# jayleicn/TVRetrieval

Hardware: AMD Instinct MI355X
Metric: queries/sec VCMR over 21.8K-video corpus (higher is better)
Workload: dtype bf16

## Files before the change

### include/xmlhip.h

```cpp
#ifndef XMLHIP_H
#define XMLHIP_H

#include <stddef.h>
#include <stdint.h>

#ifdef __cplusplus
extern "C" {
#endif

typedef void* xml_stream_t;

typedef enum { XML_F32 = 0, XML_BF16 = 1, XML_F16 = 2, XML_F16S = 3 } xml_dtype;
#define XML_F16_UNIT_LOG2 14

typedef enum {
  XML_OK = 0,
  XML_ERR_BAD_ARG = -1,
  XML_ERR_UNSUPPORTED = -2,
  XML_ERR_WORKSPACE = -3,
  XML_ERR_LAUNCH = -4
} xml_status;

int xml_abi_version(void);
const char* xml_build_arch(void);
// ... 239 lines not shown
                                    xml_stream_t stream);
int xml_q2c_scores_arg(const void* qn, const void* cn, const float* mask, float* out, int64_t ld_out, int32_t* arg,
                       int64_t ld_arg, int nq, int nv, int l, int hidden, int combine, int dt, xml_stream_t stream);
int xml_loss_combine(const float* st_ed, const float* rank2, float w_st_ed, float w_neg_ctx, float w_neg_q, float* parts4,
                     float* overall, xml_stream_t stream);
int xml_loss_combine_bwd(const float* g, float w_st_ed, float w_neg_ctx, float w_neg_q, float* d_st_ed, float* d_rank2,
                         xml_stream_t stream);
int xml_pair_sim(const void* q, const void* f2, float* sim, int64_t n, int l, int hidden, int dt,
                 xml_stream_t stream);
int xml_pair_sim_bwd(const void* q, const void* f2, const float* dsim, void* dq, void* df2, int64_t n, int l,
                     int hidden, int dt, xml_stream_t stream);
int xml_span_loss(const float* sim0, const float* sim1, const float* conv_w, const float* mask0,
                  const float* mask1, const int64_t* st_ed, int merged, int n_sim, int ks, int n, int l,
                  const float* gout, float* loss_out, float* dsim0, float* dsim1, float* dconv_w,
                  xml_stream_t stream);
int xml_rank_loss(const float* scores, const int* ranks_ctx, const int* ranks_q, float margin, int lse,
                  int n, const float* gout, float* losses, float* dscores, xml_stream_t stream);
int xml_dropout(const void* x, void* y, int64_t n, float p, uint64_t seed, const uint64_t* seed_dev, int dt,
                xml_stream_t stream);
int xml_transpose_segments(const float* src, const int64_t* table, int n_ent, int max_tiles, int dt, xml_stream_t stream);
int xml_add_layernorm_drop(const void* a, int a_dt, const void* b, const float* g, const float* beta, void* y,
                           int64_t rows, int d, int dt, float p_in, uint64_t seed_in, float p_out, uint64_t seed_out,
                           const uint64_t* seed_dev, xml_stream_t stream);
int xml_layernorm_bwd_drop(const void* a, int a_dt, const void* b, const float* g, const void* dy, void* dx, void* dxa,
                           float* dg, float* dbeta, int64_t rows, int d, int dt, float p_in, uint64_t seed_in, float p_out,
                           uint64_t seed_out, const uint64_t* seed_dev, xml_stream_t stream);
size_t xml_layernorm_bwd_partials_bytes(int64_t rows, int d);
int xml_layernorm_bwd_drop_ws(const void* a, int a_dt, const void* b, const float* g, const void* dy, void* dx, void* dxa,
                              float* dg, float* dbeta, int64_t rows, int d, int dt, float p_in, uint64_t seed_in, float p_out,
                              uint64_t seed_out, const uint64_t* seed_dev, void* ws, size_t ws_bytes, xml_stream_t stream);
int xml_clip_grad_norm(float* g, int64_t n, float max_norm, float* ws, xml_stream_t stream);
#define XML_ADAM_NORM_BLOCK 1024
int xml_bert_adam_step(float* p, float* g, float* m, float* v, const int64_t* seg_off, const float* seg_lr,
                       const float* seg_wd, int n_seg, int64_t total, float lr_mult, float b1, float b2,
                       float eps, float max_grad_norm, float* norms, const uint8_t* seg_active,
                       const float* seg_lr_mult, float* norm_ws, xml_stream_t stream);

typedef void* xml_comm_t;
int xml_rccl_available(void);
int xml_rccl_unique_id(void* id128);
int xml_rccl_comm_init(xml_comm_t* comm, int nranks, int rank, const void* id128);
int xml_rccl_comm_destroy(xml_comm_t comm);
int xml_rccl_allgather(xml_comm_t comm, const void* send, void* recv, int64_t bytes_per_rank, xml_stream_t stream);
int xml_rccl_allreduce_avg_f32(xml_comm_t comm, float* buf, int64_t n, xml_stream_t stream);
size_t xml_rccl_allgather_topk_workspace_bytes(int world, int nq, int c);
int xml_rccl_allgather_topk(xml_comm_t comm, int world, const float* loc_score, const int32_t* loc_id, int nq, int c,
                            int k, float alpha, float* out_val, int32_t* out_id, void* ws, size_t ws_bytes,
                            xml_stream_t stream);
size_t xml_rccl_topk_by_owner_workspace_bytes(int world, int per, int c);
int xml_rccl_topk_by_owner(xml_comm_t comm, int world, int rank, const float* loc_score, const int32_t* loc_id,
                           int nq, int c, int k, float alpha, float* own_val, int32_t* own_id, void* ws,
                           size_t ws_bytes, xml_stream_t stream);

size_t xml_merge_shard_topk_workspace_bytes(int world, int n_rows, int c);
int xml_merge_shard_topk(const float* recv_score, const int32_t* recv_id, int world, int n_rows, int c, int k, float alpha,
                         float* out_val, int32_t* out_id, void* ws, size_t ws_bytes, xml_stream_t stream);

int xml_index_put_rows(int n_mod, const void* f1_a, const void* f2_a, const float* mask_a, const void* f1_b,
                       const void* f2_b, const float* mask_b, const int32_t* slots, const int32_t* ids, int b, int lb,
                       void* k6_a, void* feat2_a, float* imask_a, int32_t* bits_a, void* k6_b, void* feat2_b,
                       float* imask_b, int32_t* bits_b, int32_t* vlen, int32_t* slot_ids, int32_t* live, int capacity,
                       int lpad, int l_ref, int hidden, int dt, int tiled, xml_stream_t stream);
int xml_index_clear_rows(int n_mod, const int32_t* slots, int n, float* imask_a, int32_t* bits_a, float* imask_b,
                         int32_t* bits_b, int32_t* vlen, int32_t* live, int capacity, int lpad, int l_ref,
                         xml_stream_t stream);

int xml_nms_vcmr_host(const int64_t* vid, const double* st, const double* ed, const double* score, int n,
                      double thd, int max_before, int max_after, int32_t* out_index, int32_t* n_out);
int xml_nms_svmr_host(const double* st, const double* ed, const double* score, int n, double thd,
                      int max_before, int max_after, int32_t* out_index, int32_t* n_out);
int xml_nms_vcmr_batched_host(const int64_t* vid, const double* st, const double* ed, const double* score,
                              const int32_t* count, int nq, int64_t ld, double thd, int max_before, int max_after,
                              int32_t* out_index, int64_t ld_out, int32_t* out_count, int n_threads);
int xml_nms_svmr_batched_host(const double* st, const double* ed, const double* score, const int32_t* count, int nq,
                              int64_t ld, double thd, int max_before, int max_after, int32_t* out_index, int64_t ld_out,
                              int32_t* out_count, int n_threads);

typedef enum { XML_GEMM_SMALL = 0, XML_GEMM_256 = 1, XML_GEMM_256P = 2 } xml_gemm_kernel;
typedef enum {
  XML_GEMM_FEW = 1,
  XML_GEMM_256_OK = 2,
  XML_GEMM_256P_OK = 4,
  XML_GEMM_LN_FUSED = 8,
  XML_GEMM_TILE32 = 32, XML_GEMM_TILE64 = 64, XML_GEMM_TILE128 = 128
} xml_gemm_rules;
typedef enum { XML_KLOOP_PLAIN = 1, XML_KLOOP_DEEP2 = 2, XML_KLOOP_DEEP3 = 3 } xml_gemm_kloop;
typedef enum { XML_Q2C_UNSUPPORTED = 0, XML_Q2C_STAGED = 1, XML_Q2C_RING = 2, XML_Q2C_PERSIST = 3, XML_Q2C_NONE = 4 } xml_q2c_kernel;
typedef enum { XML_Q2C_WALK_QSH = 0, XML_Q2C_WALK_TILES_PER_WORKGROUP = 1, XML_Q2C_WALK_RING_SLOTS = 2 } xml_q2c_walk;
typedef enum {
  XML_ATTN_SMALL = 0, XML_ATTN_LARGE = 1, XML_ATTN_REFUSED_HEADS = 2, XML_ATTN_REFUSED_LENGTH = 3,
  XML_ATTN_REFUSED_LDS = 4, XML_ATTN_REFUSED_DH = 5
} xml_attn_kernel;
typedef enum { XML_L2N_SCALAR = 0, XML_L2N_VEC16 = 1 } xml_l2norm_kernel;
typedef enum {
  XML_DC_SLICE_BYTES = 0,
  XML_DC_RING_SLOTS,
  XML_DC_RING_SLOTS_NOMASK,
  XML_DC_RING_LEAD,
  XML_DC_LDS_BYTES,
  XML_DC_GEMM_FEW_TILES, XML_DC_GEMM256P_MIN_TILES, XML_DC_GEMM_LN_MIN_ROWS, XML_DC_GEMM_MIN_K_BYTES,
  XML_DC_GEMM256_MIN_M, XML_DC_GEMM256_MIN_N,
  XML_DC_GEMM_TILE128_MIN_WG, XML_DC_GEMM_TILE64_MIN_WG,
  XML_DC_Q2C_PERSIST_MIN_K_BYTES,
  XML_DC_L2N_MAXJ, XML_DC_L2N_LANES,
  XML_DC_ATTN_MAX_L, XML_DC_ATTN_SMALL_MAX_L, XML_DC_ATTN_SMALL_UNITS,
  XML_DC_ATTN_N_HEAD_SIZES, XML_DC_ATTN_HEAD_SIZE0
} xml_dispatch_constant;
int64_t xml_dispatch_const(int which);
int xml_dispatch_gemm(int64_t M, int N, int K, int dt);
int xml_dispatch_gemm_rules(int64_t M, int N, int K, int dt);
int xml_dispatch_gemm_kloop(int K, int dt, int tile);
int xml_dispatch_q2c(int lpad, int hidden, int dt, int combine);
int xml_dispatch_q2c_fused(int n_mod, int lpad, int hidden, int dt, int launch);
int xml_dispatch_q2c_walk(int what, int a, int b);
int xml_dispatch_attention(int lq, int lk, int hidden, int n_heads, int dt);
int xml_dispatch_l2norm(int d, int dt);

#ifdef __cplusplus
}
#endif
#endif
```

### tvretrieval_amd/csrc/api.hip

```cpp
#include "common.h"

extern "C" int xml_abi_version(void) {
  return 6; }
extern "C" const char* xml_build_arch(void) { return "gfx950"; }
extern "C" const char* xml_status_string(int status) {
  switch (status) {
    case XML_OK: return "ok";
    case XML_ERR_BAD_ARG: return "bad argument";
    case XML_ERR_UNSUPPORTED: return "unsupported shape";
    case XML_ERR_WORKSPACE: return "workspace too small";
    case XML_ERR_LAUNCH: return "kernel launch failed";
    default: return "unknown status";
  }
}

extern "C" int64_t xml_dispatch_const(int which) {
  namespace d = dispatch;
  static const int64_t v[] = {
      d::SLICE_BYTES, d::RING_SLOTS, d::RING_SLOTS_NOMASK, d::RING_LEAD, d::LDS_BYTES, d::GEMM_FEW_TILES, d::GEMM256P_MIN_TILES,
      d::GEMM_LN_MIN_ROWS, d::GEMM_MIN_K_BYTES, d::GEMM256_MIN_M, d::GEMM256_MIN_N, d::GEMM_TILE128_MIN_WG, d::GEMM_TILE64_MIN_WG,
      d::Q2C_PERSIST_MIN_K_BYTES, d::L2N_MAXJ, d::L2N_LANES, d::ATTN_MAX_L, d::ATTN_SMALL_MAX_L, d::ATTN_SMALL_UNITS,
      d::ATTN_N_HEAD_SIZES};
  static_assert(sizeof(v) / sizeof(v[0]) == XML_DC_ATTN_HEAD_SIZE0, "one value per xml_dispatch_constant");
  if (which >= 0 && which < XML_DC_ATTN_HEAD_SIZE0) return v[which];
  const int i = which - XML_DC_ATTN_HEAD_SIZE0;
  return i >= 0 && i < d::ATTN_N_HEAD_SIZES ? d::ATTN_HEAD_SIZES[i] : -1;
}
static bool gemm_args_ok(int64_t M, int N, int K, int dt) {
  return M > 0 && N > 0 && K > 0 && (dt == XML_F32 || dt == XML_BF16 || dt == XML_F16S);
}
extern "C" int xml_dispatch_gemm(int64_t M, int N, int K, int dt) {
  return gemm_args_ok(M, N, K, dt) ? (int)dispatch::gemm_kernel(M, N, K, dt) : -1;
}
extern "C" int xml_dispatch_gemm_rules(int64_t M, int N, int K, int dt) {
  if (!gemm_args_ok(M, N, K, dt)) return -1;
  const int tile = dispatch::gemm_small_tile(M, N);
  if (dt == XML_F16S) return tile | (dispatch::gemm256_f16s_ok(M, N, 3 * K) ? XML_GEMM_256_OK : 0);
  return tile | (dispatch::gemm_few(M, N) ? XML_GEMM_FEW : 0) | (dispatch::gemm256_ok(M, N, K, dt) ? XML_GEMM_256_OK : 0) |
         (dispatch::gemm256p_ok(M, N, K, dt) ? XML_GEMM_256P_OK : 0) | (dispatch::gemm_ln_fused(M, N, K, dt) ? XML_GEMM_LN_FUSED : 0);
}
extern "C" int xml_dispatch_gemm_kloop(int K, int dt, int tile) {
  if (K <= 0 || (tile != 32 && tile != 64 && tile != 128) || !gemm_args_ok(1, 1, K, dt)) return -1;
  if (dt == XML_F16S) return XML_KLOOP_PLAIN;
  return dispatch::gemm_small_deep(tile, false) ? dispatch::gemm_small_kloop(K * (int)dt_size(dt)) : XML_KLOOP_PLAIN;
}
extern "C" int xml_dispatch_q2c(int lpad, int hidden, int dt, int combine) {
  return lpad <= 0 || hidden <= 0 || !dispatch::q2c_dt_ok(dt) ? -1 : dispatch::q2c_kernel(lpad, hidden, dt, combine != 0);
}
extern "C" int xml_dispatch_q2c_fused(int n_mod, int lpad, int hidden, int dt, int launch) {
  if (n_mod < 1 || n_mod > 2 || launch < 0 || lpad <= 0 || hidden <= 0 || !dispatch::q2c_dt_ok(dt)) return -1;
  return dispatch::q2c_fused_kernel(n_mod, lpad, hidden, dt, launch);
}
extern "C" int xml_dispatch_q2c_walk(int what, int a, int b) {
  if (what == XML_Q2C_WALK_RING_SLOTS) return a < 0 || a > 1 || b < 0 || b > 3 ? -1 : dispatch::q2c_ring_slots(a != 0, b);
  if (a <= 0 || b <= 0) return -1;
  const int tq = dispatch::q2c_tq(a), tc = dispatch::q2c_tc(b);
  if (what == XML_Q2C_WALK_QSH) return dispatch::q2c_qsh(tq, tc);
  if (what == XML_Q2C_WALK_TILES_PER_WORKGROUP) return dispatch::q2c_tiles_per_workgroup(tq, tc);
  return -1;
}
extern "C" int xml_dispatch_attention(int lq, int lk, int hidden, int n_heads, int dt) {
  const bool ok = lq > 0 && lk > 0 && hidden > 0 && (dt == XML_F32 || dt == XML_BF16);
  return ok ? dispatch::attn_kernel(lq, lk, hidden, n_heads, dt) : -1;
}
extern "C" int xml_dispatch_l2norm(int d, int dt) {
  return d <= 0 || (dt != XML_F32 && dt != XML_BF16) ? -1 : dispatch::l2n_vec_ok(d, dt) ? XML_L2N_VEC16 : XML_L2N_SCALAR;
}
```

### tvretrieval_amd/csrc/dispatch.h

```cpp
#pragma once
#include <stddef.h>
#include <stdint.h>

#include "../../include/xmlhip.h"

namespace dispatch {

constexpr int cdiv(int64_t a, int64_t b) { return (int)((a + b - 1) / b); }
constexpr size_t dt_size(int dt) { return (dt == XML_F32 || dt == XML_F16S) ? 4 : 2; }
constexpr size_t max_of(size_t a, size_t b) { return a > b ? a : b; }

constexpr int LDS_BYTES = 160 * 1024;
constexpr int SLICE_BYTES = 64;
constexpr int RING_SLOTS = 4;
constexpr int RING_SLOTS_NOMASK = 5;
constexpr int RING_LEAD = 5;
constexpr int RING_ROWS = 256;

constexpr int GEMM_FEW_TILES = 64;
constexpr int GEMM256P_MIN_TILES = 3072;
constexpr int64_t GEMM_LN_MIN_ROWS = 2048;
constexpr int GEMM_MIN_K_BYTES = 256;
constexpr int GEMM256_MIN_M = 256, GEMM256_MIN_N = 128;
constexpr int GEMM_TILE128_MIN_WG = 512, GEMM_TILE64_MIN_WG = 192;
constexpr int GEMM_SMALL_STEP_BYTES = 128;

constexpr int64_t gemm_tiles(int64_t M, int N) { return (int64_t)cdiv(M, 256) * cdiv(N, 256); }
constexpr bool gemm_few(int64_t M, int N) { return gemm_tiles(M, N) < GEMM_FEW_TILES; }
constexpr bool gemm_ring_k(size_t k_bytes) { return k_bytes % (2 * SLICE_BYTES) == 0 && k_bytes >= GEMM_MIN_K_BYTES; }
constexpr bool gemm256_ok(int64_t M, int N, int K, int dt) {
  return M >= GEMM256_MIN_M && N >= GEMM256_MIN_N && gemm_ring_k((size_t)K * dt_size(dt));
}
constexpr bool gemm256_f16s_ok(int64_t M, int N, int K3) {
  return M >= GEMM256_MIN_M && N >= GEMM256_MIN_N && N % 8 == 0 && gemm_ring_k((size_t)K3 * 2);
}
constexpr bool gemm256p_ok(int64_t M, int N, int K, int dt) {
  return gemm_ring_k((size_t)K * dt_size(dt)) && N >= GEMM256_MIN_N && N % 8 == 0 && gemm_tiles(M, N) >= GEMM256P_MIN_TILES;
}
constexpr bool gemm_ln_fused(int64_t M, int N, int K, int dt) {
  return (dt == XML_F32 || dt == XML_BF16) && gemm_ring_k((size_t)K * dt_size(dt)) && N % 256 == 0 && N / 256 <= 3 &&
         M >= GEMM_LN_MIN_ROWS;
}
constexpr xml_gemm_kernel gemm_kernel(int64_t M, int N, int K, int dt) {
  if (dt == XML_F16S) return gemm256_f16s_ok(M, N, 3 * K) ? XML_GEMM_256 : XML_GEMM_SMALL;
  if (!gemm_few(M, N) && gemm256p_ok(M, N, K, dt)) return XML_GEMM_256P;
  if (!gemm_few(M, N) && gemm256_ok(M, N, K, dt)) return XML_GEMM_256;
  return XML_GEMM_SMALL;
}
constexpr int gemm_small_tile(int64_t M, int N) {
  const int64_t wg128 = (int64_t)cdiv(N, 128) * cdiv(M, 128);
  return wg128 >= GEMM_TILE128_MIN_WG ? 128 : wg128 * 4 >= GEMM_TILE64_MIN_WG ? 64 : 32;
}
constexpr bool gemm_small_deep(int tile, bool f16_operands) { return tile < 128 && !f16_operands; }
template <typename D3, typename D2, typename P>
constexpr void gemm_small_kloop_run(int k_bytes, D3&& deep3, D2&& deep2, P&& plain) {
  const int nsteps = (k_bytes + GEMM_SMALL_STEP_BYTES - 1) / GEMM_SMALL_STEP_BYTES;
  if (nsteps % 3 == 0) deep3();
  else if (nsteps % 2 == 0) deep2();
  else plain();
}
constexpr xml_gemm_kloop gemm_small_kloop(int k_bytes) {
  xml_gemm_kloop r = XML_KLOOP_PLAIN;
  gemm_small_kloop_run(k_bytes, [&] { r = XML_KLOOP_DEEP3; }, [&] { r = XML_KLOOP_DEEP2; }, [] {});
  return r;
}

constexpr int Q2C_PERSIST_MIN_K_BYTES = 384;
constexpr bool q2c_dt_ok(int dt) { return dt == XML_F32 || dt == XML_BF16 || dt == XML_F16; }
constexpr bool q2c_shape_ok(int lpad, int hidden) { return lpad % 16 == 0 && lpad <= 128 && hidden % 8 == 0; }
constexpr bool q2c_tiled_ok(int lpad, int hidden, int dt) {
  const size_t kb = (size_t)hidden * dt_size(dt);
  return q2c_dt_ok(dt) && lpad == 128 && kb % (2 * SLICE_BYTES) == 0 && kb >= Q2C_PERSIST_MIN_K_BYTES;
}
constexpr bool q2c_persist_ok(int lpad, int hidden, int dt) { return dt != XML_F16 && q2c_tiled_ok(lpad, hidden, dt); }
constexpr bool q2c_ring_ok(int hidden, int dt) { return dt != XML_F16 && ((size_t)hidden * dt_size(dt)) % (2 * SLICE_BYTES) == 0; }
constexpr xml_q2c_kernel q2c_kernel(int lpad, int hidden, int dt, bool combine) {
  if (!q2c_shape_ok(lpad, hidden)) return XML_Q2C_UNSUPPORTED;
  if (q2c_persist_ok(lpad, hidden, dt) && !combine) return XML_Q2C_PERSIST;
  return q2c_ring_ok(hidden, dt) ? XML_Q2C_RING : XML_Q2C_STAGED;
}
constexpr xml_q2c_kernel q2c_fused_kernel(int n_mod, int lpad, int hidden, int dt, int launch) {
  if (!q2c_shape_ok(lpad, hidden)) return launch == 0 ? XML_Q2C_UNSUPPORTED : XML_Q2C_NONE;
  if (q2c_persist_ok(lpad, hidden, dt)) return launch == 0 ? XML_Q2C_PERSIST : XML_Q2C_NONE;
  return launch < n_mod ? q2c_kernel(lpad, hidden, dt, launch > 0) : XML_Q2C_NONE;
}
constexpr int q2c_tq(int nq) { return cdiv(nq, 256); }
constexpr int q2c_tc(int nv) { return cdiv(nv, 2); }
constexpr int64_t q2c_walk_slots(int tq, int tc, int qsh) {
  const int64_t qg = (tq + (1 << qsh) - 1) >> qsh, per = 8ll << (5 - qsh);
  return (qg << qsh) * ((tc + per - 1) / per * per);
}
constexpr int q2c_qsh(int tq, int tc) {
  const int qsh = tq >= 5 ? 3 : tq >= 3 ? 2 : tq == 2 ? 1 : 0;
  return qsh == 3 && q2c_walk_slots(tq, tc, 2) * 100 < q2c_walk_slots(tq, tc, 3) * 97 ? 2 : qsh;
}
constexpr int q2c_tiles_per_workgroup(int tq, int tc) {
  const int qsh = q2c_qsh(tq, tc);
  return cdiv(tq, 1 << qsh) * cdiv(tc, 8 << (5 - qsh));
}
constexpr int q2c_ring_slots(bool tiled, int mask_mode) {
  return tiled && (mask_mode == 1 || mask_mode == 2) ? RING_SLOTS_NOMASK : RING_SLOTS;
}

constexpr int L2N_MAXJ = 8, L2N_LANES = 32;
constexpr bool l2n_vec_ok(int d, int dt) {
  const int vec = 16 / (int)dt_size(dt);
  return (dt == XML_F32 || dt == XML_BF16) && d % vec == 0 && d / vec <= L2N_LANES * L2N_MAXJ;
}
constexpr bool tile_rows_l2norm_ok(int hidden, int dt) {
  return hidden > 0 && l2n_vec_ok(hidden, dt) && (hidden * (int)dt_size(dt)) % SLICE_BYTES == 0;
}

#define XML_ATTN_HEAD_SIZES(X) X(32) X(64) X(96) X(128) X(192)
#define XML_ATTN_LIST(D) D,
constexpr int ATTN_HEAD_SIZES[] = {XML_ATTN_HEAD_SIZES(XML_ATTN_LIST)};
#undef XML_ATTN_LIST
constexpr int ATTN_N_HEAD_SIZES = sizeof(ATTN_HEAD_SIZES) / sizeof(ATTN_HEAD_SIZES[0]);
constexpr int ATTN_MAX_L = 128;
constexpr int ATTN_SMALL_MAX_L = 32;
constexpr int ATTN_SMALL_UNITS = 4;
constexpr bool attn_head_size_ok(int dh) {
  for (int i = 0; i < ATTN_N_HEAD_SIZES; ++i)
    if (ATTN_HEAD_SIZES[i] == dh) return true;
  return false;
// ... 32 lines not shown
```

### tvretrieval_amd/csrc/gemm256p.hip

```cpp
#include <type_traits>

#include "internal.h"
#include "ring256.h"

struct G256pArgs {
  const void* A;
  const void* W;
  const float* bias;
  const void* addend;
  void* out;
  int64_t M, n_tiles;
  int N, K, relu, add_mode, seq_len, tn;
  float* ln_scratch;
  const float* ln_g;
  const float* ln_b;
  float ln_eps;
  int probe;
};

#ifdef XML_DEBUG_VARIANTS
__device__ unsigned long long g_g256p_probe[8 * 8];
__device__ unsigned int g_g256p_steps[8 * 64];
extern "C" int xml_debug_read_gemm_steps(unsigned int* host_out) {
  return hipMemcpyFromSymbol(host_out, HIP_SYMBOL(g_g256p_steps), sizeof(unsigned int) * 512) == hipSuccess ? 0 : -4;
// ... 479 lines not shown
#pragma unroll
            for (int m4 = 0; m4 < 4; ++m4) {
              const int lr64 = m4 * 16 + fr_e;
              const float mean = patch[lr64 * 2], rstd = patch[lr64 * 2 + 1];
              int boff = fg_e * GC;
              asm volatile("" : "+v"(boff));
              float x[NGRP * GC];
              if (t == tn_s - 1) {
#pragma unroll
                for (int q = 0; q < NGRP; ++q)
#pragma unroll
                  for (int e = 0; e < GC; ++e)
                    x[q * GC + e] = PAIRED ? acc[m4][2 * q + (e >> 2)][e & 3] : acc[m4][q][e & 3];
              } else {
#pragma unroll
                for (int j = 0; j < 8; ++j) {
                  typedef float xml_nt4 __attribute__((ext_vector_type(4)));
                  const xml_nt4 f = __builtin_nontemporal_load(reinterpret_cast<const xml_nt4*>(sc + (m4 * 8 + j) * 512));
                  x[j * 4] = f.x; x[j * 4 + 1] = f.y; x[j * 4 + 2] = f.z; x[j * 4 + 3] = f.w;
                }
              }
              float v[NGRP][GC];
#pragma unroll
              for (int q = 0; q < NGRP; ++q)
#pragma unroll
                for (int e = 0; e < GC; e += 4) {
                  const float4 g4 = *reinterpret_cast<const float4*>(patch + 384 + q * (4 * GC) + boff + e);
                  const float4 b4 = *reinterpret_cast<const float4*>(patch + 512 + q * (4 * GC) + boff + e);
                  const float gq[4] = {g4.x, g4.y, g4.z, g4.w}, bq[4] = {b4.x, b4.y, b4.z, b4.w};
#pragma unroll
                  for (int j = 0; j < 4; ++j) v[q][e + j] = (x[q * GC + e + j] - mean) * rstd * gq[j] + bq[j];
                }
              store_rows(m4, v, (t - nt) * 256);
            }
          }
          __builtin_amdgcn_s_waitcnt(0xc07f);
          __builtin_amdgcn_wave_barrier();
        }
      }
    }
    { const unsigned long long t = G256P_T(); pr[4] += t - pt; pt = t; }
    ++pr[6];
    ++c_k;
    if (tile_of(c_k) >= a.n_tiles) break;
  }
#ifdef XML_DEBUG_VARIANTS
  if ((a.probe & 1) && blockIdx.x == 0 && lane == 0) {
    pr[5] = __builtin_amdgcn_s_memtime() - pr_t0;
    pr[7] = __builtin_amdgcn_s_memrealtime() - pr_r0;
    for (int i = 0; i < 8; ++i) g_g256p_probe[wave * 8 + i] = pr[i];
    for (int i = 0; i < 64; ++i) g_g256p_steps[wave * 64 + i] = sp[i];
  }
#endif
  };
  if (grp) run(std::true_type{});
  else run(std::false_type{});
  asm volatile("s_waitcnt vmcnt(0)" ::: "memory");
  __builtin_amdgcn_s_barrier();
}

template <typename T, typename OutT, typename AddT, bool LNE = false, bool DIRECT = true>
static int launch_gemm256p(const void* A, const void* W, const float* bias, const void* addend, void* out, int64_t M,
                           int N, int K, int relu, int add_mode, int seq_len, hipStream_t st, const float* ln_g = nullptr,
                           const float* ln_b = nullptr, void* ln_ws = nullptr) {
  G256pArgs a;
  a.A = A; a.W = W; a.bias = bias; a.addend = addend; a.out = out;
  a.M = M; a.N = N; a.K = K; a.relu = relu; a.add_mode = add_mode; a.seq_len = seq_len;
  a.tn = cdiv(N, 256);
  a.n_tiles = (int64_t)cdiv(M, 256) * a.tn;
  a.ln_scratch = (float*)ln_ws; a.ln_g = ln_g; a.ln_b = ln_b; a.ln_eps = 1e-5f;
  a.probe = g_q2c_ablation == 9 ? 1 : g_q2c_ablation == 21 ? 2 : g_q2c_ablation == 22 ? 4 : g_q2c_ablation == 23 ? 6 : g_q2c_ablation == 24 ? 8 : 0;
  const int lds = dispatch::RING_SLOTS * ring256::SLOT_BYTES + 8 * 4096;
#ifdef XML_DEBUG_VARIANTS
  if (!LNE && DIRECT && g_gemm_variant == 3)
    return launch_gemm256p<T, OutT, AddT, false, false>(A, W, bias, addend, out, M, N, K, relu, add_mode, seq_len, st);
#endif
  auto kern = gemm256p_kernel<T, OutT, AddT, LNE, DIRECT>;
  if (!xml_lds_attr_once<gemm256p_kernel<T, OutT, AddT, LNE, DIRECT>>(lds)) return XML_ERR_LAUNCH;
  hipLaunchKernelGGL(kern, dim3(256), dim3(512), lds, st, a);
  XML_CHECK_LAUNCH();
  return XML_OK;
}

size_t xmli_gemm_ln_workspace_bytes(int64_t M, int N) {
  (void)M;
  return align_up((size_t)256 * (size_t)(N / 256 > 1 ? N / 256 - 1 : 0) * 256 * 256 * 4 + 256, 256);
}
int xmli_gemm_ln(const void* A, const void* W, const float* bias, const void* addend, const float* ln_g, const float* ln_b,
                 void* y, int64_t M, int N, int K, int relu, int add_mode, int seq_len, int dt, void* ln_ws,
                 hipStream_t st) {
  if (!ln_ws) return XML_ERR_WORKSPACE;
  if (dt == XML_F32)
    return launch_gemm256p<float, float, float, true>(A, W, bias, addend, y, M, N, K, relu, add_mode, seq_len, st, ln_g,
                                                      ln_b, ln_ws);
  return launch_gemm256p<bf16_t, bf16_t, bf16_t, true>(A, W, bias, addend, y, M, N, K, relu, add_mode, seq_len, st, ln_g,
                                                        ln_b, ln_ws);
}

template <typename OutT, int TN>
__global__ __launch_bounds__(64) void ln_lne_order_kernel(const float* __restrict__ pre, const float* __restrict__ ln_g,
                                                           const float* __restrict__ ln_b, OutT* __restrict__ y,
                                                           int64_t rows, int N, float ln_eps) {
#pragma clang fp contract(off)
  constexpr int GC = sizeof(OutT) == 2 ? 8 : 4;
  constexpr int NGRP = 128 / (4 * GC);
  constexpr int LPR = TN == 1 ? 8 : TN == 2 ? 16 : 32;
  const int lane = threadIdx.x & 63;
  const int sub = lane & (LPR - 1);
  const int base = lane - sub;
  const int64_t row = ((int64_t)blockIdx.x * 64 + threadIdx.x) / LPR;
  if (row >= rows || sub >= 8 * TN) return;
  const int seg = sub >> 2, fg = sub & 3;
  const int c0 = (seg >> 1) * 256 + (seg & 1) * 128 + fg * GC;
  const float* pr = pre + row * N;
  float v[NGRP][GC], gv[NGRP][GC], bv[NGRP][GC];
#pragma unroll
  for (int q = 0; q < NGRP; ++q)
#pragma unroll
    for (int e = 0; e < GC; e += 4) {
      const float4 f = *reinterpret_cast<const float4*>(pr + c0 + q * (4 * GC) + e);
      const float4 g4 = *reinterpret_cast<const float4*>(ln_g + c0 + q * (4 * GC) + e);
      const float4 b4 = *reinterpret_cast<const float4*>(ln_b + c0 + q * (4 * GC) + e);
      v[q][e] = f.x; v[q][e + 1] = f.y; v[q][e + 2] = f.z; v[q][e + 3] = f.w;
      gv[q][e] = g4.x; gv[q][e + 1] = g4.y; gv[q][e + 2] = g4.z; gv[q][e + 3] = g4.w;
      bv[q][e] = b4.x; bv[q][e + 1] = b4.y; bv[q][e + 2] = b4.z; bv[q][e + 3] = b4.w;
    }
#pragma unroll
  for (int q = 0; q < NGRP; ++q)
#pragma unroll
    for (int e = 0; e < GC; ++e) asm volatile("" : "+v"(v[q][e]), "+v"(gv[q][e]), "+v"(bv[q][e]));
  float s = 0.f;
#pragma unroll
  for (int q = 0; q < NGRP; ++q)
#pragma unroll
    for (int e = 0; e < GC; ++e) s += v[q][e];
  s += __shfl_xor(s, 1, 64);
  s += __shfl_xor(s, 2, 64);
  const float* vf = &v[0][0];
  const float cs0 = __builtin_fmaf(s, -1.0f / 128.0f, vf[0]), cs1 = __builtin_fmaf(s, -1.0f / 128.0f, vf[1]);
  float c2 = __builtin_fmaf(cs0, cs0, cs1 * cs1);
#pragma unroll
  for (int k = 2; k < NGRP * GC; ++k) {
    const float c = __builtin_fmaf(s, -1.0f / 128.0f, vf[k]);
    c2 = __builtin_fmaf(c, c, c2);
  }
  c2 += __shfl_xor(c2, 1, 64);
  c2 += __shfl_xor(c2, 2, 64);
  typedef float xml_f4 __attribute__((ext_vector_type(4)));
  xml_f4 pv[3];
#pragma unroll
  for (int t = 0; t < 3; ++t)
    pv[t] = t < TN ? xml_f4{__shfl(s, base + t * 8, 64), __shfl(c2, base + t * 8, 64), __shfl(s, base + t * 8 + 4, 64),
                            __shfl(c2, base + t * 8 + 4, 64)}
                   : xml_f4{0.f, 0.f, 0.f, 0.f};
  float tot = 0.f;
#pragma unroll
  for (int t = 0; t < 3; ++t) tot += pv[t].x + pv[t].z;
  const float mean = tot / (float)N;
  float m2 = 0.f;
#pragma unroll
  for (int t = 0; t < TN; ++t) {
    const float d0 = __builtin_fmaf(pv[t].x, 1.0f / 128.0f, -mean), d1 = __builtin_fmaf(pv[t].z, 1.0f / 128.0f, -mean);
    float u = __builtin_fmaf(d0, 128.0f * d0, pv[t].y);
    u = pv[t].w + u;
    u = __builtin_fmaf(d1, 128.0f * d1, u);
    m2 = u + m2;
  }
  const float rstd = 1.0f / sqrtf(m2 / (float)N + ln_eps);
#pragma unroll
  for (int q = 0; q < NGRP; ++q) {
    float o[GC];
#pragma unroll
    for (int e = 0; e < GC; ++e) o[e] = __builtin_fmaf((v[q][e] - mean) * rstd, gv[q][e], bv[q][e]);
    st_global16(y + row * N + c0 + q * (4 * GC), pack16<OutT>(o));
  }
}

int xmli_gemm_ln_tail(const float* pre, const float* ln_g, const float* ln_b, void* y, int64_t M, int N, int dt,
                      hipStream_t st) {
  const int tn = N / 256;
// ... 25 lines not shown
```

Before: 147,300.

## Add register-resident 128-row GEMM+LayerNorm kernel for bf16 narrow rows

Adds a persistent GEMM kernel that computes 128-row blocks across all 1-2 column tiles, keeping the accumulators in registers so LayerNorm statistics and normalization happen in-kernel. It replaces the previous fused path, which spilled partial tiles to a float workspace, for bf16 shapes with N=512 or small-M N=256. The goal is to avoid the workspace round-trip and the cross-tile reduction traffic. The costs are much higher register pressure, a fixed grid of 256 workgroups, and a more complex pipelined ring schedule.

```diff
diff --git a/include/xmlhip.h b/include/xmlhip.h
--- a/include/xmlhip.h
+++ b/include/xmlhip.h
@@ -345,6 +345,7 @@
   XML_GEMM_256_OK = 2,
   XML_GEMM_256P_OK = 4,
   XML_GEMM_LN_FUSED = 8,
+  XML_GEMM_LN_REGS = 16,
   XML_GEMM_TILE32 = 32, XML_GEMM_TILE64 = 64, XML_GEMM_TILE128 = 128
 } xml_gemm_rules;
 typedef enum { XML_KLOOP_PLAIN = 1, XML_KLOOP_DEEP2 = 2, XML_KLOOP_DEEP3 = 3 } xml_gemm_kloop;
diff --git a/tvretrieval_amd/csrc/api.hip b/tvretrieval_amd/csrc/api.hip
--- a/tvretrieval_amd/csrc/api.hip
+++ b/tvretrieval_amd/csrc/api.hip
@@ -37,7 +37,8 @@
   const int tile = dispatch::gemm_small_tile(M, N);
   if (dt == XML_F16S) return tile | (dispatch::gemm256_f16s_ok(M, N, 3 * K) ? XML_GEMM_256_OK : 0);
   return tile | (dispatch::gemm_few(M, N) ? XML_GEMM_FEW : 0) | (dispatch::gemm256_ok(M, N, K, dt) ? XML_GEMM_256_OK : 0) |
-         (dispatch::gemm256p_ok(M, N, K, dt) ? XML_GEMM_256P_OK : 0) | (dispatch::gemm_ln_fused(M, N, K, dt) ? XML_GEMM_LN_FUSED : 0);
+         (dispatch::gemm256p_ok(M, N, K, dt) ? XML_GEMM_256P_OK : 0) | (dispatch::gemm_ln_fused(M, N, K, dt) ? XML_GEMM_LN_FUSED : 0) |
+         (dispatch::gemm_ln_regs(M, N, K, dt) ? XML_GEMM_LN_REGS : 0);
 }
 extern "C" int xml_dispatch_gemm_kloop(int K, int dt, int tile) {
   if (K <= 0 || (tile != 32 && tile != 64 && tile != 128) || !gemm_args_ok(1, 1, K, dt)) return -1;
diff --git a/tvretrieval_amd/csrc/dispatch.h b/tvretrieval_amd/csrc/dispatch.h
--- a/tvretrieval_amd/csrc/dispatch.h
+++ b/tvretrieval_amd/csrc/dispatch.h
@@ -40,6 +40,13 @@
 constexpr bool gemm_ln_fused(int64_t M, int N, int K, int dt) {
   return (dt == XML_F32 || dt == XML_BF16) && gemm_ring_k((size_t)K * dt_size(dt)) && N % 256 == 0 && N / 256 <= 3 &&
          M >= GEMM_LN_MIN_ROWS;
+}
+constexpr int GEMM_LN_REGS_ROWS = 128;
+constexpr int GEMM_LN_REGS_MAX_TN = 2;
+constexpr int GEMM_LN_WORKGROUPS = 256;
+constexpr bool gemm_ln_regs(int64_t M, int N, int K, int dt) {
+  return gemm_ln_fused(M, N, K, dt) && dt == XML_BF16 &&
+         (N / 256 == 2 || (N / 256 == 1 && (M + GEMM_LN_REGS_ROWS - 1) / GEMM_LN_REGS_ROWS <= GEMM_LN_WORKGROUPS));
 }
 constexpr xml_gemm_kernel gemm_kernel(int64_t M, int N, int K, int dt) {
   if (dt == XML_F16S) return gemm256_f16s_ok(M, N, 3 * K) ? XML_GEMM_256 : XML_GEMM_SMALL;
diff --git a/tvretrieval_amd/csrc/gemm256p.hip b/tvretrieval_amd/csrc/gemm256p.hip
--- a/tvretrieval_amd/csrc/gemm256p.hip
+++ b/tvretrieval_amd/csrc/gemm256p.hip
@@ -585,6 +585,343 @@
   return XML_OK;
 }
 
+template <typename T, int TN>
+__global__ __launch_bounds__(512) void gemm128ln_kernel(G256pArgs a) {
+#pragma clang fp contract(off)
+  static_assert(sizeof(T) == 2 && TN >= 1 && TN <= 3, "2-byte operands, rows of 1-3 column tiles");
+  using namespace ring256;
+  constexpr int NSLOT = dispatch::RING_SLOTS;
+  constexpr int RING_BYTES = NSLOT * SLOT_BYTES;
+  constexpr int N = TN * 256;
+  constexpr int RB = dispatch::GEMM_LN_REGS_ROWS;
+  extern __shared__ __attribute__((aligned(16))) char smem[];
+
+  const int tid = threadIdx.x, lane = tid & 63;
+  const int wave = __builtin_amdgcn_readfirstlane(tid >> 6);
+  const int wm = wave >> 1, wn = wave & 1;
+  const int grp = wave >> 2;
+  const int fr = lane & 15, fg = lane >> 4;
+  const int k_bytes = a.K * (int)sizeof(T);
+  const int n_slices = k_bytes / ROWB;
+  const T* A = reinterpret_cast<const T*>(a.A);
+  const T* W = reinterpret_cast<const T*>(a.W);
+  const T* addend = reinterpret_cast<const T*>(a.addend);
+  T* out = reinterpret_cast<T*>(a.out);
+  const int64_t M = a.M;
+  const int64_t n_rb = a.n_tiles;
+  auto rb_of = [&](int i) -> int64_t { return (int64_t)i * dispatch::GEMM_LN_WORKGROUPS + blockIdx.x; };
+
+  const uint32_t lds0 = (uint32_t)(uintptr_t)(__attribute__((address_space(3))) char*)smem;
+  int i_rb = 0, i_nt = 0, i_slice = 0, i_slot = 0, i_left = n_slices, i_inc = 1;
+  uint32_t va[2] = {}, vb[2] = {};
+  const char* sbase_a = nullptr;
+  const char* sbase_b = nullptr;
+  auto setup_issue_tile = [&]() {
+    const int64_t m0 = rb_of(i_rb) * RB;
+    const int n0 = i_nt * 256;
+    const int lane_o = ring_lane_now();
+    const int rsub = lane_o >> 2, pslot = lane_o & 3;
+    auto off_a = [&](int piece) -> uint32_t {
+      const int row = piece * 16 + rsub;
+      return (uint32_t)((m0 + row < M) ? row : 0) * k_bytes + (pslot ^ ring_swz(row)) * 16;
+    };
+    auto off_b = [&](int piece) -> uint32_t {
+      const int row = piece * 16 + rsub;
+      return (uint32_t)row * k_bytes + (pslot ^ ring_swz(row)) * 16;
+    };
+    if (grp == 0) {
+      va[0] = off_a(wave * 2); va[1] = off_a(wave * 2 + 1);
+      vb[0] = off_b(wave * 2); vb[1] = off_b(wave * 2 + 1);
+    } else {
+      vb[0] = off_b(8 + (wave - 4) * 2); vb[1] = off_b(9 + (wave - 4) * 2);
+    }
+    sbase_a = reinterpret_cast<const char*>(A) + m0 * k_bytes;
+    sbase_b = reinterpret_cast<const char*>(W) + (int64_t)n0 * k_bytes;
+  };
+  auto issue_slice = [&]() {
+    const int koff = i_slice * ROWB;
+    const uint32_t slot0 = lds0 + i_slot * SLOT_BYTES;
+    if (grp == 0) {
+      ring_dma_pair(va[0], va[1], sbase_a + koff, slot0 + wave * 2048);
+      ring_dma_pair(vb[0], vb[1], sbase_b + koff, slot0 + OPER_BYTES + wave * 2048);
+    } else {
+      ring_dma_pair(vb[0], vb[1], sbase_b + koff, slot0 + OPER_BYTES + 8192 + (wave - 4) * 2048);
+    }
+    if (++i_slot == NSLOT) i_slot = 0;
+    i_slice += i_inc;
+    if (--i_left == 0) {
+      i_slice = 0;
+      i_left = n_slices;
+      if (++i_nt == TN) { i_nt = 0; ++i_rb; }
+      if (rb_of(i_rb) < n_rb) setup_issue_tile();
+      else { i_left = 0x7fffffff; i_inc = 0; }
+    }
+  };
+  if (rb_of(0) >= n_rb) return;
+  setup_issue_tile();
+
+  const int a_off = (wm * 32 + fr) * ROWB + ((fg ^ ring_swz(fr)) << 4);
+  const int rb_e = (fr >> 2) * 8 + (fr & 3);
+  const int b_off = OPER_BYTES + (wn * 128 + rb_e) * ROWB + ((fg ^ ring_swz(rb_e)) << 4);
+  const int b_off_o = OPER_BYTES + (wn * 128 + rb_e + 4) * ROWB + ((fg ^ ring_swz(rb_e + 4)) << 4);
+  auto b_frag = [&](const char* slot, int n) -> uint4 {
+    return *reinterpret_cast<const uint4*>(slot + ((n & 1) ? b_off_o : b_off) + (n >> 1) * 32 * ROWB);
+  };
+  int c_rb = 0, c_slot = 0;
+  issue_slice(); issue_slice(); issue_slice(); issue_slice();
+  if (grp == 0) asm volatile("s_waitcnt vmcnt(12)" ::: "memory");
+  else asm volatile("s_waitcnt vmcnt(6)" ::: "memory");
+  __builtin_amdgcn_s_barrier();
+
+  uint4 faA[2], faB[2], fbL[4], fbH[4];
+  constexpr int GC = 8, NGRP = 4;
+
+  auto run = [&](auto grp_tag) {
+  constexpr bool GRP1 = decltype(grp_tag)::value;
+  for (;;) {
+    f32x4 acc[TN][2][8];
+    const int64_t m0 = rb_of(c_rb) * RB;
+    const uint32_t m0_mod = a.add_mode == 1 ? (uint32_t)(m0 % a.seq_len) : 0u;
+#pragma unroll
+    for (int t = 0; t < TN; ++t) {
+      {
+        const char* slot0 = smem + c_slot * SLOT_BYTES;
+#pragma unroll
+        for (int m = 0; m < 2; ++m) faA[m] = *reinterpret_cast<const uint4*>(slot0 + a_off + m * 16 * ROWB);
+#pragma unroll
+        for (int n = 0; n < 4; ++n) fbL[n] = b_frag(slot0, n);
+      }
+      auto slice_step = [&](uint4 (&fc)[2], uint4 (&fn)[2], auto init_tag) {
+        constexpr bool INIT = decltype(init_tag)::value;
+        const char* slot = smem + c_slot * SLOT_BYTES;
+#pragma unroll
+        for (int n = 0; n < 4; ++n) fbH[n] = b_frag(slot, n + 4);
+#pragma unroll
+        for (int m = 0; m < 2; ++m)
+#pragma unroll
+          for (int n = 0; n < 4; ++n) {
+            if constexpr (INIT) RingInit<T>::chunk(acc[t][m][n], fbL[n], fc[m]);
+            else Mma<T>::chunk(acc[t][m][n], fbL[n], fc[m]);
+          }
+        if (!GRP1) __builtin_amdgcn_s_waitcnt(0x0078);
+        else __builtin_amdgcn_s_waitcnt(0x0074);
+        __builtin_amdgcn_s_barrier();
+        if (++c_slot == NSLOT) c_slot = 0;
+        auto next_reads = [&]() {
+          const char* nslot = smem + c_slot * SLOT_BYTES;
+#pragma unroll
+          for (int m = 0; m < 2; ++m) fn[m] = *reinterpret_cast<const uint4*>(nslot + a_off + m * 16 * ROWB);
+#pragma unroll
+          for (int n = 0; n < 4; ++n) fbL[n] = b_frag(nslot, n);
+        };
+        if (!GRP1) { next_reads(); issue_slice(); }
+        __builtin_amdgcn_sched_barrier(0);
+#pragma unroll
+        for (int m = 0; m < 2; ++m)
+#pragma unroll
+          for (int n = 0; n < 4; ++n) {
+            if constexpr (INIT) RingInit<T>::chunk(acc[t][m][n + 4], fbH[n], fc[m]);
+            else Mma<T>::chunk(acc[t][m][n + 4], fbH[n], fc[m]);
+          }
+        __builtin_amdgcn_sched_barrier(0);
+        if (GRP1) { next_reads(); issue_slice(); }
+      };
+      slice_step(faA, faB, std::true_type{});
+      slice_step(faB, faA, std::false_type{});
+      for (int s2 = 2; s2 < n_slices; s2 += 2) {
+        slice_step(faA, faB, std::false_type{});
+        slice_step(faB, faA, std::false_type{});
+      }
+
+      const int lane_e = ring_lane_now();
+      const int fr_e = lane_e & 15, fg_e = lane_e >> 4;
+      float* patch = reinterpret_cast<float*>(smem + RING_BYTES) + wave * 1024;
+      {
+        float4 b4 = make_float4(0.f, 0.f, 0.f, 0.f);
+        if (a.bias) b4 = *reinterpret_cast<const float4*>(a.bias + t * 256 + wn * 128 + (lane_e & 31) * 4);
+        __builtin_amdgcn_wave_barrier();
+        if (lane_e < 32) *reinterpret_cast<float4*>(patch + 256 + lane_e * 4) = b4;
+        __builtin_amdgcn_s_waitcnt(0xc07f);
+        __builtin_amdgcn_wave_barrier();
+      }
+#pragma unroll
+      for (int m = 0; m < 2; ++m) {
+        const int lrow = wm * 32 + m * 16 + fr_e;
+        uint4 ad[NGRP];
+        if (a.add_mode) {
+          const bool rok = m0 + lrow < M;
+          const int64_t arow = a.add_mode == 1 ? (int64_t)((m0_mod + (uint32_t)lrow) % (uint32_t)a.seq_len) : m0 + lrow;
+          const T* ap = addend + arow * N + t * 256 + wn * 128 + fg_e * GC;
+#pragma unroll
+          for (int q = 0; q < NGRP; ++q) ad[q] = rok ? ld_global16(ap + q * (4 * GC)) : make_uint4(0u, 0u, 0u, 0u);
+        }
+        int boff = fg_e * GC;
+        asm volatile("" : "+v"(boff));
+#pragma unroll
+        for (int q = 0; q < NGRP; ++q) {
+          float gb[GC];
+#pragma unroll
+          for (int e = 0; e < GC; e += 4) {
+            const float4 b4 = *reinterpret_cast<const float4*>(patch + 256 + q * (4 * GC) + boff + e);
+            gb[e] = b4.x; gb[e + 1] = b4.y; gb[e + 2] = b4.z; gb[e + 3] = b4.w;
+          }
+#pragma unroll
+          for (int e = 0; e < GC; ++e) {
+            float x = acc[t][m][2 * q + (e >> 2)][e & 3] + gb[e];
+            if (a.relu) x = fmaxf(x, 0.f);
+            acc[t][m][2 * q + (e >> 2)][e & 3] = x;
+          }
+        }
+        if (a.add_mode) {
+#pragma unroll
+          for (int q = 0; q < NGRP; ++q) {
+            float av[8];
+            unpack16<bf16_t>(ad[q], av);
+#pragma unroll
+            for (int e = 0; e < GC; ++e) acc[t][m][2 * q + (e >> 2)][e & 3] += av[e];
+          }
+        }
+        float s = 0.f;
+#pragma unroll
+        for (int k = 0; k < NGRP * GC; ++k) s += acc[t][m][k >> 2][k & 3];
+        s += __shfl_xor(s, 16, 64);
+        s += __shfl_xor(s, 32, 64);
+        const float cs0 = __builtin_fmaf(s, -1.0f / 128.0f, acc[t][m][0][0]);
+        const float cs1 = __builtin_fmaf(s, -1.0f / 128.0f, acc[t][m][0][1]);
+        float c2 = __builtin_fmaf(cs0, cs0, cs1 * cs1);
+#pragma unroll
+        for (int k = 2; k < NGRP * GC; ++k) {
+          const float c = __builtin_fmaf(s, -1.0f / 128.0f, acc[t][m][k >> 2][k & 3]);
+          c2 = __builtin_fmaf(c, c, c2);
+        }
+        c2 += __shfl_xor(c2, 16, 64);
+        c2 += __shfl_xor(c2, 32, 64);
+        if (fg_e == 0) {
+          float* ps = patch + 640 + ((m * 16 + fr_e) * TN + t) * 2;
+          ps[0] = s;
+          ps[1] = c2;
+        }
+        asm volatile("" ::: "memory");
+      }
+    }
+
+    {
+      const int lane_e = ring_lane_now();
+      const int fr_e = lane_e & 15, fg_e = lane_e >> 4;
+      float* patch = reinterpret_cast<float*>(smem + RING_BYTES) + wave * 1024;
+      __builtin_amdgcn_s_waitcnt(0xc07f);
+      __builtin_amdgcn_s_barrier();
+      {
+        const float* p0 = reinterpret_cast<const float*>(smem + RING_BYTES) + (wm * 2) * 1024 + 640 + (lane_e & 31) * TN * 2;
+        const float* p1 = p0 + 1024;
+        typedef float xml_f4 __attribute__((ext_vector_type(4)));
+        xml_f4 pv[3];
+#pragma unroll
+        for (int t = 0; t < 3; ++t)
+          pv[t] = t < TN ? xml_f4{p0[t * 2], p0[t * 2 + 1], p1[t * 2], p1[t * 2 + 1]} : xml_f4{0.f, 0.f, 0.f, 0.f};
+        float tot = 0.f;
+#pragma unroll
+        for (int t = 0; t < 3; ++t) tot += pv[t].x + pv[t].z;
+        const float mean = tot / (float)a.N;
+        float m2 = 0.f;
+#pragma unroll
+        for (int t = 0; t < TN; ++t) {
+          const float d0 = __builtin_fmaf(pv[t].x, 1.0f / 128.0f, -mean), d1 = __builtin_fmaf(pv[t].z, 1.0f / 128.0f, -mean);
+          float u = __builtin_fmaf(d0, 128.0f * d0, pv[t].y);
+          u = pv[t].w + u;
+          u = __builtin_fmaf(d1, 128.0f * d1, u);
+          m2 = u + m2;
+        }
+        const float rstd = 1.0f / sqrtf(m2 / (float)a.N + a.ln_eps);
+        if (lane_e < 32) {
+          patch[lane_e * 2] = mean;
+          patch[lane_e * 2 + 1] = rstd;
+        }
+      }
+      const bool odd = (fr_e & 1) != 0;
+#pragma unroll
+      for (int t = 0; t < TN; ++t) {
+        __builtin_amdgcn_wave_barrier();
+        {
+          const int bc = t * 256 + wn * 128 + (lane_e & 31) * 4;
+          const float4 g4 = *reinterpret_cast<const float4*>(a.ln_g + bc);
+          const float4 b4 = *reinterpret_cast<const float4*>(a.ln_b + bc);
+          if (lane_e < 32) {
+            *reinterpret_cast<float4*>(patch + 384 + lane_e * 4) = g4;
+            *reinterpret_cast<float4*>(patch + 512 + lane_e * 4) = b4;
+          }
+        }
+        __builtin_amdgcn_s_waitcnt(0xc07f);
+        __builtin_amdgcn_wave_barrier();
+#pragma unroll
+        for (int m = 0; m < 2; ++m) {
+          const int lr32 = m * 16 + fr_e;
+          const float mean = patch[lr32 * 2], rstd = patch[lr32 * 2 + 1];
+          const int r_even = wm * 32 + m * 16 + (fr_e & ~1);
+          const int64_t m_even = m0 + r_even;
+          int boff = fg_e * GC;
+          asm volatile("" : "+v"(boff));
+#pragma unroll
+          for (int pq = 0; pq < NGRP / 2; ++pq) {
+            uint4 pk[2];
+#pragma unroll
+            for (int qi = 0; qi < 2; ++qi) {
+              const int q = 2 * pq + qi;
+              float o[GC];
+#pragma unroll
+              for (int e = 0; e < GC; e += 4) {
+                const float4 g4 = *reinterpret_cast<const float4*>(patch + 384 + q * (4 * GC) + boff + e);
+                const float4 b4 = *reinterpret_cast<const float4*>(patch + 512 + q * (4 * GC) + boff + e);
+                const float gq[4] = {g4.x, g4.y, g4.z, g4.w}, bq[4] = {b4.x, b4.y, b4.z, b4.w};
+#pragma unroll
+                for (int j = 0; j < 4; ++j)
+                  o[e + j] = __builtin_fmaf((acc[t][m][2 * q + (e >> 2)][j] - mean) * rstd, gq[j], bq[j]);
+              }
+              pk[qi] = pack16<T>(o);
+            }
+            const uint4 dn = ring_dpp_u4<0x111>(pk[1]);
+            const uint4 up = ring_dpp_u4<0x101>(pk[0]);
+            const uint4 d_even = make_uint4(odd ? dn.x : pk[0].x, odd ? dn.y : pk[0].y, odd ? dn.z : pk[0].z, odd ? dn.w : pk[0].w);
+            const uint4 d_odd = make_uint4(odd ? pk[1].x : up.x, odd ? pk[1].y : up.y, odd ? pk[1].z : up.z, odd ? pk[1].w : up.w);
+            const int col = t * 256 + wn * 128 + pq * (8 * GC) + (fr_e & 1) * (4 * GC) + fg_e * GC;
+            typedef unsigned int g_u4 __attribute__((ext_vector_type(4)));
+            char* ob = reinterpret_cast<char*>(out + m0 * N);
+            const uint32_t oo = (uint32_t)(r_even * N + col) * (uint32_t)sizeof(T);
+            if (m_even < M) __builtin_nontemporal_store(g_u4{d_even.x, d_even.y, d_even.z, d_even.w}, reinterpret_cast<g_u4*>(ob + oo));
+            if (m_even + 1 < M) __builtin_nontemporal_store(g_u4{d_odd.x, d_odd.y, d_odd.z, d_odd.w}, reinterpret_cast<g_u4*>(ob + oo + N * (uint32_t)sizeof(T)));
+            asm volatile("" ::: "memory");
+          }
+        }
+      }
+      __builtin_amdgcn_s_waitcnt(0xc07f);
+      __builtin_amdgcn_wave_barrier();
+    }
+    ++c_rb;
+    if (rb_of(c_rb) >= n_rb) break;
+  }
+  };
+  if (grp) run(std::true_type{});
+  else run(std::false_type{});
+  asm volatile("s_waitcnt vmcnt(0)" ::: "memory");
+  __builtin_amdgcn_s_barrier();
+}
+
+template <typename T, int TN>
+static int launch_gemm128ln(const void* A, const void* W, const float* bias, const void* addend, void* out, int64_t M, int K,
+                            int relu, int add_mode, int seq_len, hipStream_t st, const float* ln_g, const float* ln_b) {
+  G256pArgs a = {};
+  a.A = A; a.W = W; a.bias = bias; a.addend = addend; a.out = out;
+  a.M = M; a.N = TN * 256; a.K = K; a.relu = relu; a.add_mode = add_mode; a.seq_len = seq_len;
+  a.tn = TN;
+  a.n_tiles = cdiv(M, dispatch::GEMM_LN_REGS_ROWS);
+  a.ln_g = ln_g; a.ln_b = ln_b; a.ln_eps = 1e-5f;
+  const int lds = dispatch::RING_SLOTS * ring256::SLOT_BYTES + 8 * 4096;
+  if (!xml_lds_attr_once<gemm128ln_kernel<T, TN>>(lds)) return XML_ERR_LAUNCH;
+  hipLaunchKernelGGL((gemm128ln_kernel<T, TN>), dim3(dispatch::GEMM_LN_WORKGROUPS), dim3(512), lds, st, a);
+  XML_CHECK_LAUNCH();
+  return XML_OK;
+}
+
 size_t xmli_gemm_ln_workspace_bytes(int64_t M, int N) {
   (void)M;
   return align_up((size_t)256 * (size_t)(N / 256 > 1 ? N / 256 - 1 : 0) * 256 * 256 * 4 + 256, 256);
@@ -593,12 +930,46 @@
                  void* y, int64_t M, int N, int K, int relu, int add_mode, int seq_len, int dt, void* ln_ws,
                  hipStream_t st) {
   if (!ln_ws) return XML_ERR_WORKSPACE;
+  bool regs = dispatch::gemm_ln_regs(M, N, K, dt);
+#ifdef XML_DEBUG_VARIANTS
+  if (g_gemm_variant == 4) regs = false;
+#endif
+  if (regs) {
+    const int tn = N / 256;
+#define XML_LNR(TN) launch_gemm128ln<bf16_t, TN>(A, W, bias, addend, y, M, K, relu, add_mode, seq_len, st, ln_g, ln_b)
+    static_assert(dispatch::GEMM_LN_REGS_MAX_TN == 2, "one instantiation per column-tile count the rule admits");
+    return tn == 1 ? XML_LNR(1) : XML_LNR(2);
+#undef XML_LNR
+  }
   if (dt == XML_F32)
     return launch_gemm256p<float, float, float, true>(A, W, bias, addend, y, M, N, K, relu, add_mode, seq_len, st, ln_g,
                                                       ln_b, ln_ws);
   return launch_gemm256p<bf16_t, bf16_t, bf16_t, true>(A, W, bias, addend, y, M, N, K, relu, add_mode, seq_len, st, ln_g,
                                                         ln_b, ln_ws);
 }
+
+#ifdef XML_DEBUG_VARIANTS
+extern "C" size_t xml_debug_gemm_ln_workspace_bytes(int64_t M, int N) {
+  const size_t pre = align_up((size_t)M * (size_t)N * 4, 256), fused = xmli_gemm_ln_workspace_bytes(M, N);
+  return pre > fused ? pre : fused;
+}
+extern "C" int xml_debug_gemm_ln(const void* A, const void* W, const float* bias, const void* addend, const float* ln_g,
+                                 const float* ln_b, void* y, int64_t M, int N, int K, int relu, int add_mode, int seq_len,
+                                 int dt, int form, void* ws, xml_stream_t stream) {
+  if (!A || !W || !ln_g || !ln_b || !y || !ws || (add_mode && !addend) || form < 0 || form > 2) return XML_ERR_BAD_ARG;
+  if (!dispatch::gemm_ln_fused(M, N, K, dt)) return XML_ERR_UNSUPPORTED;
+  hipStream_t st = (hipStream_t)stream;
+  if (form == 2) {
+    const int rc = xmli_gemm(A, W, bias, addend, ws, M, N, K, relu, add_mode, seq_len,  1, dt, st);
+    return rc ? rc : xmli_gemm_ln_tail((const float*)ws, ln_g, ln_b, y, M, N, dt, st);
+  }
+  const int keep = g_gemm_variant;
+  if (form == 1) g_gemm_variant = 4;
+  const int rc = xmli_gemm_ln(A, W, bias, addend, ln_g, ln_b, y, M, N, K, relu, add_mode, seq_len, dt, ws, st);
+  g_gemm_variant = keep;
+  return rc;
+}
+#endif
 
 template <typename OutT, int TN>
 __global__ __launch_bounds__(64) void ln_lne_order_kernel(const float* __restrict__ pre, const float* __restrict__ ln_g,
```

New measurement: 147,500 (median of 5 runs). Within noise of the previous version (+0.1%).
